# theartful/polychase

Measured on AMD Instinct MI355X. Metric: optical-flow frames/sec, higher is better.
Workload: dtype u8/int32 fixed-point + f32 2x2 solve; 1 GPU; C2 1920x1080 300-frame synthetic clip, 3-level pyramidal LK (max_level=3); width=1920, height=1080, max_level=3, window=10, pairs_per_frame=8, frames_per_gpu=1877, arith=opencv_x86, parallelism=single GPU

## Files before the change

### include/polychase_hip.h

```cpp
#ifndef POLYCHASE_HIP_H_
#define POLYCHASE_HIP_H_

#include <stddef.h>
#include <stdint.h>

#ifdef __cplusplus
extern "C" {
#endif

#define PC_OK 0
#define PC_E_INVALID (-1)
#define PC_E_NO_DEVICE (-2)
#define PC_E_HIP (-3)
#define PC_E_CAPACITY (-4)
#define PC_E_STATE (-5)

#define PC_MAX_TARGETS 8
#define PC_MAX_LEVELS 16
#define PC_MAX_WINDOW 31

typedef struct pc_context pc_context;
typedef struct pc_frame pc_frame;

typedef struct pc_gftt_options {
// ... 118 lines not shown
#define PC_ANALYZER_SPARE_SLOTS 3
#define PC_ANALYZER_LOOKAHEAD 1
int pc_analyzer_create(pc_context* ctx, int width, int height, const pc_gftt_options* gftt,
                       const pc_flow_options* flow, int ring_frames, int max_jobs, pc_analyzer** out);
void pc_analyzer_destroy(pc_analyzer* a);
int pc_analyzer_reset(pc_analyzer* a);
int pc_analyzer_put_frame(pc_analyzer* a, int32_t frame_id, const uint8_t* rgb, size_t row_pitch,
                          int on_device, int will_detect);
int pc_analyzer_put_frame_f32(pc_analyzer* a, int32_t frame_id, const float* rgb, size_t row_pitch, int channels,
                              int on_device, int will_detect);
int pc_analyzer_has_frame(const pc_analyzer* a, int32_t frame_id);
int pc_analyzer_frame_ingested(const pc_analyzer* a, int32_t frame_id);
int pc_analyzer_set_keypoints(pc_analyzer* a, int32_t frame_id, const float* xy, int n);
int pc_analyzer_submit(pc_analyzer* a, int32_t frame1, const int32_t* targets, int n_targets);
int pc_analyzer_pending(const pc_analyzer* a);
#define PC_LOG_MAGIC 0x50434c4f47303031ll
int pc_analyzer_set_device_log(pc_analyzer* a, void* d_log, size_t capacity_bytes);
int pc_analyzer_device_log_used(const pc_analyzer* a, size_t* bytes);
int pc_analyzer_redirect_device_log(pc_analyzer* a, void* d_log, size_t capacity_bytes);
int pc_analyzer_set_host_records(pc_analyzer* a, int enabled);
int pc_analyzer_set_fb_threshold(pc_analyzer* a, double fb_threshold);
int pc_analyzer_set_mask(pc_analyzer* a, const uint8_t* mask, size_t row_pitch, int on_device);
int pc_analyzer_set_mask_polygons(pc_analyzer* a, const float* xy, const int32_t* counts, int n_polygons, int invert);
int pc_analyzer_collect(pc_analyzer* a, pc_frame_result* out);

typedef struct pc_mesh pc_mesh;
typedef struct pc_pnp_problem pc_pnp_problem;

int pc_mesh_create(pc_context* ctx, const float* vertices, int n_vertices, const uint32_t* triangles,
                   int n_triangles, pc_mesh** out);
// ... 175 lines not shown
```

### polychase_amd/csrc/hip/api_analyzer.hip

```cpp
#include "api_internal.hpp"

using namespace pc_api;


namespace {

constexpr int kSpareSlots = PC_ANALYZER_SPARE_SLOTS;

enum DetState { DET_NONE = 0, DET_ENQUEUED = 2, DET_DONE = 3 };

struct Slot {
    pc_frame* frame = nullptr;
    int32_t frame_id = 0;
    bool valid = false;
    DetState det = DET_NONE;
    bool supplied = false;
    DetectScratch scratch;
    hipEvent_t last_read[2] = {nullptr, nullptr};
    hipEvent_t img_ready = nullptr;
    hipEvent_t kps_ready = nullptr;
};

struct Job {
    int32_t frame1 = 0;
    int n_kps = 0;
    bool detected = false;
    int n_targets = 0;
    int32_t targets[PC_MAX_TARGETS];
    PinBuf<uint8_t> h_pack;
    size_t o_kps = 0, o_idx = 0, o_xy = 0, o_err = 0, pack_bytes = 0;
    bool host_records = true;
    hipEvent_t done = nullptr;
};

struct HelperPriorityControl {
    static constexpr int kCalm = 48;
    static constexpr int kLagsToRaise = 3;
    int mode = -1;
    int hi = 0;
    int calm = 0;
    uint32_t window = 0;
    uint64_t lag_seen = 0, switched_on = 0;
    void init() {
        const char* v = getenv("POLYCHASE_HELPER_PRIO");
        mode = (v && (v[0] == '0' || v[0] == '1') && v[1] == 0) ? v[0] - '0' : -1;
        hi = mode == 1 ? 1 : 0;
    }
    void observe(bool lagging) {
        if (mode >= 0) return;
        window = ((window << 1) | (lagging ? 1u : 0u)) & 0xffffu;
        if (lagging) {
            lag_seen++;
            calm = 0;
            if (!hi && __builtin_popcount(window) >= kLagsToRaise) {
                hi = 1;
                switched_on++;
            }
        } else if (hi && ++calm >= kCalm) {
            hi = 0;
            calm = 0;
            window = 0;
        }
    }
};
struct HelperPriorityScope {
    explicit HelperPriorityScope(int hi) { pc::set_helper_prio(hi); }
    ~HelperPriorityScope() { pc::set_helper_prio(0); }
};

}

struct pc_analyzer {
    pc_context* ctx = nullptr;
    int w = 0, h = 0;
    pc_gftt_options gopt;
    pc_flow_options fopt;
    pc::GfttGrid grid;
    std::vector<Slot> slots;
    std::vector<Job> jobs;
    size_t job_head = 0, job_count = 0;
    uint64_t submitted = 0;
    bool one_lane = false;
    static constexpr int kLaneEvents = 16;
    hipEvent_t lk_done[2][kLaneEvents] = {};
    bool gate_armed = false;
    HelperPriorityControl prio;
    int32_t put_newest = 0, put_previous = 0;
    int puts = 0;
    bool host_records = true;
    double fb_threshold = 0.0;
    static constexpr int kMaskGens = 4;
    int mask_kind = 0;
    int mask_gen = 0;
    PinBuf<uint8_t> mask_host[kMaskGens];
    hipEvent_t mask_copied[kMaskGens] = {};
    const uint8_t* mask_dev = nullptr;
    size_t mask_dev_pitch = 0;
    int poly_gen = 0, poly_vertices = 0, poly_polygons = 0, poly_invert = 0;
    PinBuf<int32_t> poly_host[kMaskGens];
    DevBuf<int32_t> poly_dev[kMaskGens];
    hipEvent_t poly_read[kMaskGens] = {};
    uint8_t* d_log = nullptr;
    size_t log_cap = 0, log_used = 0;
// ... 8 lines not shown
    return (s.valid && s.frame_id == frame_id) ? &s : nullptr;
}

int detect_dense(pc_analyzer* a, Slot& s) {
    hipStream_t const ds = a->ctx->detect_stream_for(s.frame_id);
    PrepScope prep(a->ctx, ds);
    if (ds != a->ctx->prep_stream) PC_HIP(hipStreamWaitEvent(ds, s.img_ready, 0));
    int rc = detect_enqueue(a->ctx, s.frame, a->grid, a->gopt, s.scratch, s.scratch.bin_hist);
    if (rc != PC_OK) return rc;
    PC_HIP(hipEventRecord(s.kps_ready, ds));
    s.det = DET_ENQUEUED;
    s.supplied = false;
    return PC_OK;
}

int detect_finish_slot(pc_analyzer* a, Slot& s) {
    int rc;
    if (s.det == DET_NONE && (rc = detect_dense(a, s)) != PC_OK) return rc;
    {
        hipStream_t const ds = a->ctx->detect_stream_for(s.frame_id);
        PrepScope prep(a->ctx, ds);
        bool redone = false;
        if ((rc = detect_finish(a->ctx, s.frame, a->grid, a->gopt, s.scratch, s.scratch.bin_hist, &redone)) != PC_OK) return rc;
        if (redone) PC_HIP(hipEventRecord(s.kps_ready, ds));
    }
    s.det = DET_DONE;
    return PC_OK;
}

}

extern "C" {
// ... 7 lines not shown
    pc::GfttGrid grid0;
    {
        int vrc = validate_gftt(gftt, width, height, &grid0);
        if (vrc != PC_OK) return vrc;
    }
    PC_HIP(hipSetDevice(ctx->device));
    pc_analyzer* a = new (std::nothrow) pc_analyzer();
    if (!a) return fail(PC_E_INVALID, "out of host memory");
    a->ctx = ctx;
    a->one_lane = getenv("POLYCHASE_LK_LANES") && atoi(getenv("POLYCHASE_LK_LANES")) == 1;
    a->w = width;
    a->h = height;
    a->gopt = *gftt;
    a->fopt = *flow;
    a->grid = grid0;
    a->prio.init();
    a->slots.resize((size_t)ring_frames + kSpareSlots);
    a->jobs.resize((size_t)max_jobs);
    int rc = PC_OK;
    for (auto& s : a->slots) {
        rc = pc_frame_create(ctx, width, height, flow->window_size, flow->max_level, &s.frame);
        if (rc != PC_OK) break;
        const int kp0 = std::max(16384, (width * height) / 16);
        if ((rc = ensure_kp_capacity(s.frame, kp0)) != PC_OK) break;
        if (hipMalloc(reinterpret_cast<void**>(&s.frame->d_perm), (size_t)kp0 * 2 * sizeof(uint32_t)) != hipSuccess) {
            rc = fail(PC_E_HIP, "hipMalloc failed");
            break;
        }
        s.frame->perm_cap = kp0;
        if ((rc = detect_reserve(ctx, width, height, s.scratch, &a->gopt)) != PC_OK) break;
        if (s.scratch.bin_hist.ensure((size_t)pc::bin_num_tiles(width, height) + 1) != hipSuccess) {
// ... 81 lines not shown
    for (auto& s : a->slots) {
        s.valid = false;
        s.det = DET_NONE;
        s.supplied = false;
        s.frame_id = 0;
        s.last_read[0] = s.last_read[1] = nullptr;
        s.scratch.cleared = false;
        if (s.frame) s.frame->mask_on = false;
    }
    a->mask_kind = 0;
    a->mask_dev = nullptr;
    a->job_head = 0;
    a->d_log = nullptr;
    a->log_cap = a->log_used = 0;
    a->host_records = true;
    a->put_newest = a->put_previous = 0;
    a->puts = 0;
    a->prio = HelperPriorityControl();
    a->prio.init();
    return PC_OK;
}

static int analyzer_put(pc_analyzer* a, int32_t frame_id, const uint8_t* rgb, size_t row_pitch, int on_device,
                        int will_detect, int channels, int elem_size) {
    if (!a || !rgb) return fail(PC_E_INVALID, "null argument");
    const int n = (int)a->slots.size();
    Slot& s = a->slots[(size_t)(((frame_id % n) + n) % n)];
    PC_HIP(hipSetDevice(a->ctx->device));
    PrepScope prep(a->ctx);
    HelperPriorityScope prio_scope(a->prio.hi);
    a->put_previous = a->put_newest;
    a->put_newest = frame_id;
    a->puts++;
    for (hipEvent_t& e : s.last_read) {
        if (e) PC_HIP(hipStreamWaitEvent(a->ctx->prep_stream, e, 0));
        e = nullptr;
    }
    if (s.valid && s.det == DET_ENQUEUED && a->ctx->n_detect > 0) PC_HIP(hipStreamWaitEvent(a->ctx->prep_stream, s.kps_ready, 0));
    const bool clear_here = will_detect && a->ctx->n_detect == 0;
    int rc = set_image(a->ctx, s.frame, rgb, row_pitch, on_device, channels, elem_size, clear_here ? s.scratch.counters.p : nullptr,
                       detect_counter_words(s.scratch));
    s.scratch.cleared = rc == PC_OK && clear_here;
    if (rc != PC_OK) {
        s.valid = false;
        return rc;
    }
    s.frame->mask_on = false;
    if (will_detect && a->mask_kind == 1) {
// ... 1 lines not shown
        if ((rc = upload_mask(s.frame, a->mask_host[g].p, (size_t)a->w, PC_FRAME_PINNED_HOST, a->ctx->prep_stream)) != PC_OK) return rc;
        PC_HIP(hipEventRecord(a->mask_copied[g], a->ctx->prep_stream));
    } else if (will_detect && a->mask_kind == 2) {
        if ((rc = upload_mask(s.frame, a->mask_dev, a->mask_dev_pitch, 1, a->ctx->prep_stream)) != PC_OK) return rc;
    } else if (will_detect && a->mask_kind == 3) {
        const int g = a->poly_gen;
        if ((rc = fill_mask_polygons(s.frame, a->poly_dev[g].p, a->poly_vertices, a->poly_polygons, a->poly_invert, a->ctx->prep_stream)) != PC_OK)
            return rc;
        PC_HIP(hipEventRecord(a->poly_read[g], a->ctx->prep_stream));
    }
    PC_HIP(hipEventRecord(s.img_ready, a->ctx->prep_stream));
    s.frame_id = frame_id;
    s.valid = true;
    s.det = DET_NONE;
    s.supplied = false;
    if (will_detect) return detect_dense(a, s);
    return PC_OK;
}

int pc_analyzer_put_frame(pc_analyzer* a, int32_t frame_id, const uint8_t* rgb, size_t row_pitch, int on_device,
                          int will_detect) {
    return analyzer_put(a, frame_id, rgb, row_pitch, on_device, will_detect, 3, 1);
}

int pc_analyzer_put_frame_f32(pc_analyzer* a, int32_t frame_id, const float* rgb, size_t row_pitch, int channels,
                              int on_device, int will_detect) {
    return analyzer_put(a, frame_id, reinterpret_cast<const uint8_t*>(rgb), row_pitch, on_device, will_detect, channels, 4);
}

int pc_analyzer_has_frame(const pc_analyzer* a, int32_t frame_id) {
    if (!a) return 0;
    return find_slot(const_cast<pc_analyzer*>(a), frame_id) != nullptr;
}

int pc_analyzer_frame_ingested(const pc_analyzer* a, int32_t frame_id) {
    if (!a) return 1;
    Slot* s = find_slot(const_cast<pc_analyzer*>(a), frame_id);
    if (!s || !s->img_ready) return 1;
    return hipEventQuery(s->img_ready) == hipSuccess ? 1 : 0;
}

int pc_analyzer_set_keypoints(pc_analyzer* a, int32_t frame_id, const float* xy, int n) {
    if (!a || n < 0 || (!xy && n > 0)) return fail(PC_E_INVALID, "bad argument");
    Slot* s = find_slot(a, frame_id);
    if (!s) return fail(PC_E_STATE, "frame %d is not resident", frame_id);
    HelperPriorityScope prio_scope(a->prio.hi);
    int rc = ensure_kp_capacity(s->frame, n);
    if (rc != PC_OK) return rc;
    if (n > 0) {
        hipStream_t const ds = a->ctx->detect_stream_for(frame_id);
        PC_HIP(hipStreamSynchronize(ds));
        PC_HIP(hipMemcpyAsync(s->frame->d_kps, xy, (size_t)n * sizeof(float2), hipMemcpyHostToDevice, ds));
        PC_HIP(hipStreamSynchronize(ds));
    }
    s->frame->n_kps = n;
    {
        hipStream_t const ds = a->ctx->detect_stream_for(frame_id);
        PrepScope prep(a->ctx, ds);
        if ((rc = order_keypoints_spatially(a->ctx, s->frame, s->scratch.bin_hist)) != PC_OK) return rc;
        PC_HIP(hipEventRecord(s->kps_ready, ds));
    }
    s->det = DET_DONE;
    s->supplied = true;
    return PC_OK;
}


int pc_analyzer_submit(pc_analyzer* a, int32_t frame1, const int32_t* targets, int n_targets) {
    if (!a || (n_targets > 0 && !targets)) return fail(PC_E_INVALID, "null argument");
    if (n_targets < 0 || n_targets > PC_MAX_TARGETS) return fail(PC_E_INVALID, "n_targets must be in [0,%d]", PC_MAX_TARGETS);
    if (a->job_count == a->jobs.size()) return fail(PC_E_STATE, "%zu jobs already in flight: call pc_analyzer_collect", a->job_count);
    pc_context* ctx = a->ctx;
    PC_HIP(hipSetDevice(ctx->device));
    HelperPriorityScope prio_scope(a->prio.hi);
    Slot* s1 = find_slot(a, frame1);
    if (!s1) return fail(PC_E_STATE, "frame1 %d is not resident", frame1);
    const pc_frame* tg[PC_MAX_TARGETS];
    for (int t = 0; t < n_targets; t++) {
        Slot* st = find_slot(a, targets[t]);
        if (!st) return fail(PC_E_STATE, "target frame %d is not resident", targets[t]);
        tg[t] = st->frame;
    }
    int rc;
    bool detected = false;
    if (s1->det != DET_DONE) {
        SlowSection ss("submit/detect_finish");
        if ((rc = detect_finish_slot(a, *s1)) != PC_OK) return rc;
        detected = true;
    } else {
// ... 82 lines not shown
        hh[1] = frame1;
        hh[2] = n;
        hh[3] = n_targets;
        for (int t = 0; t < n_targets; t++) hh[4 + t] = targets[t];
        hh[12] = (long long)rows;
        PC_HIP(hipMemcpyAsync(a->d_log + o_hdr, hh, 128, hipMemcpyHostToDevice, ls));
        PC_HIP(hipMemcpyAsync(a->d_log + o_hdr + 128, pack, j.pack_bytes, hipMemcpyDeviceToDevice, ls));
        a->log_used = end;
    }
    a->submitted++;
    if (a->host_records) PC_HIP(hipMemcpyAsync(j.h_pack.p, pack, j.pack_bytes, hipMemcpyDeviceToHost, ls));
    else PC_HIP(hipMemcpyAsync(j.h_pack.p, pack, 128, hipMemcpyDeviceToHost, ls));
    j.host_records = a->host_records;
    PC_HIP(hipEventRecord(j.done, ls));
    a->job_count++;
    return PC_OK;
}

int pc_analyzer_pending(const pc_analyzer* a) { return a ? (int)a->job_count : 0; }

int pc_analyzer_set_device_log(pc_analyzer* a, void* d_log, size_t capacity_bytes) {
    if (!a) return fail(PC_E_INVALID, "null analyzer");
    if (d_log && (reinterpret_cast<uintptr_t>(d_log) & 15)) return fail(PC_E_INVALID, "device log must be 16-byte aligned");
    PC_HIP(a->ctx->sync_side_streams());
    PC_HIP(hipStreamSynchronize(a->ctx->stream));
    a->d_log = static_cast<uint8_t*>(d_log);
    a->log_cap = d_log ? capacity_bytes : 0;
    a->log_used = 0;
    return PC_OK;
}

int pc_analyzer_redirect_device_log(pc_analyzer* a, void* d_log, size_t capacity_bytes) {
    if (!a || !d_log) return fail(PC_E_INVALID, "null argument");
    if (reinterpret_cast<uintptr_t>(d_log) & 15) return fail(PC_E_INVALID, "device log must be 16-byte aligned");
// ... 72 lines not shown
    a->mask_dev = nullptr;
    return PC_OK;
}

int pc_analyzer_device_log_used(const pc_analyzer* a, size_t* bytes) {
    if (!a || !bytes) return fail(PC_E_INVALID, "null argument");
    *bytes = a->log_used;
    return PC_OK;
}

int pc_analyzer_collect(pc_analyzer* a, pc_frame_result* out) {
    if (!a || !out) return fail(PC_E_INVALID, "null argument");
    if (a->job_count == 0) return fail(PC_E_STATE, "no job in flight");
    Job& j = a->jobs[a->job_head];
    PC_HIP(hipEventSynchronize(j.done));
    if (a->puts >= 2) {
        Slot* const sp = find_slot(a, a->put_previous);
        bool lagging = sp && sp->img_ready && hipEventQuery(sp->img_ready) == hipErrorNotReady;
        if (a->ctx->n_detect > 0 && !lagging) {
            Slot* const sd = find_slot(a, j.frame1 + (int32_t)a->job_count + 1);
            lagging = sd && sd->det == DET_ENQUEUED && sd->kps_ready && hipEventQuery(sd->kps_ready) == hipErrorNotReady;
        }
        a->prio.observe(lagging);
    }
    (void)hipStreamQuery(a->ctx->stream);
    if (a->ctx->stream_b) (void)hipStreamQuery(a->ctx->stream_b);
    (void)hipStreamQuery(a->ctx->prep_stream);
    for (int k = 0; k < a->ctx->n_detect; k++) (void)hipStreamQuery(a->ctx->detect_stream[k]);
    out->frame1 = j.frame1;
    out->n_keypoints = j.n_kps;
    out->keypoints_detected = j.detected ? 1 : 0;
    out->keypoints_xy = j.host_records ? reinterpret_cast<const float*>(j.h_pack.p + j.o_kps) : nullptr;
    out->n_targets = j.n_targets;
    for (int t = 0; t < PC_MAX_TARGETS; t++) out->targets[t] = t < j.n_targets ? j.targets[t] : 0;
    const long long* h_ro = reinterpret_cast<const long long*>(j.h_pack.p);
    for (int t = 0; t <= PC_MAX_TARGETS; t++) out->row_offset[t] = (int64_t)h_ro[std::min(t, j.n_targets)];
    out->src_indices = j.host_records ? reinterpret_cast<const uint32_t*>(j.h_pack.p + j.o_idx) : nullptr;
    out->tgt_xy = j.host_records ? reinterpret_cast<const float*>(j.h_pack.p + j.o_xy) : nullptr;
// ... 8 lines not shown
```

### polychase_amd/csrc/hip/kernels.hpp

```cpp
#pragma once

#include "bvh.hpp"
#include "common.hpp"

namespace pc {

int helper_prio_arg();
void set_helper_prio(int hi);

void launch_rgb2gray(const uint8_t* rgb, size_t rgb_pitch, const Level& l0, hipStream_t s);
void launch_rgbf32_to_gray(const float* rgb, size_t rgb_pitch, int channels, const Level& l0, hipStream_t s);
void launch_copy_gray(const uint8_t* gray, size_t gray_pitch, const Level& l0, hipStream_t s);
void launch_pyrdown(const Level& src, const Level& dst, hipStream_t s);
void launch_border(const Level& l, int win, hipStream_t s);
void launch_widen(const Level& l, int win, hipStream_t s);
void launch_scharr(const Level& l, hipStream_t s);

enum LevelSourceKind { SRC_PYR = 0, SRC_RGB8 = 1, SRC_GRAY8 = 2, SRC_RGBF32 = 3 };
struct LevelSource {
    int kind;
    const uint8_t* src;
    size_t src_pitch;
    int channels;
    int aligned;
// ... 229 lines not shown
```

### polychase_amd/csrc/hip/kernels_gftt.hip

```cpp
#include <algorithm>
#include <cstring>
#include <type_traits>
#include <rocprim/device/device_radix_sort.hpp>

#include <cmath>

#include "kernels.hpp"

namespace pc {

constexpr int TW = 64, TH = 16;
constexpr int GH = TH + 4, G_PITCH = 72;
constexpr int CW = TW + 2, CH = TH + 2;

template <bool ROW_FMA>
__device__ __forceinline__ float smooth_row(float a, float b, float c, float f1, float f0) {
    float t = f1 * a;
    if (ROW_FMA) {
        t = __fmaf_rn(f0, b, t);
        t = __fmaf_rn(f1, c, t);
    } else {
        t += f0 * b;
        t += f1 * c;
    }
// ... 317 lines not shown

static int min_eig_variant() {
    static const int v = [] {
        const char* e = getenv("POLYCHASE_MINEIG_VARIANT");
        return e ? atoi(e) : 0;
    }();
    return v;
}

template <int SOBEL, bool MASKED>
static void launch_min_eig_masked(const Level& l0, float* eig, const GfttGrid& g, uint32_t* cell_max, float f1, float f0, hipStream_t s,
                                  const uint8_t* mask) {
    if (min_eig_variant() == 0) {
        dim3 grid2((l0.w + 2 * ME_TW - 1) / (2 * ME_TW), (l0.h + 2 * ME_TH - 1) / (2 * ME_TH));
        hipLaunchKernelGGL((min_eig_fused_kernel<SOBEL, MASKED>), grid2, dim3(256), 0, s, l0.img, l0.pitch, l0.w, l0.h, eig, g, cell_max, f1, f0,
                           helper_prio_arg(), mask);
        return;
    }
    dim3 grid((l0.w + TW - 1) / TW, (l0.h + TH - 1) / TH);
    hipLaunchKernelGGL((min_eig_kernel<SOBEL, MASKED>), grid, dim3(256), 0, s, l0.img, l0.pitch, l0.w, l0.h, eig, g, cell_max, f1, f0,
                       helper_prio_arg(), mask);
}
template <int SOBEL>
static void launch_min_eig_mode(const Level& l0, float* eig, const GfttGrid& g, uint32_t* cell_max, float f1, float f0, hipStream_t s,
                                const uint8_t* mask) {
    if (mask) launch_min_eig_masked<SOBEL, true>(l0, eig, g, cell_max, f1, f0, s, mask);
    else launch_min_eig_masked<SOBEL, false>(l0, eig, g, cell_max, f1, f0, s, nullptr);
}
void launch_min_eig(const Level& l0, float* eig, const GfttGrid& g, uint32_t* cell_max, int sobel_fma, hipStream_t s, const uint8_t* mask) {
    const double scale_d = 1.0 / (4.0 * 3.0 * 255.0);
    const float f1 = (float)(1.0 * scale_d), f0 = (float)(2.0 * scale_d);
    switch (sobel_fma & 3) {
        case 0: launch_min_eig_mode<0>(l0, eig, g, cell_max, f1, f0, s, mask); break;
        case 1: launch_min_eig_mode<1>(l0, eig, g, cell_max, f1, f0, s, mask); break;
        case 2: launch_min_eig_mode<2>(l0, eig, g, cell_max, f1, f0, s, mask); break;
        default: launch_min_eig_mode<3>(l0, eig, g, cell_max, f1, f0, s, mask); break;
// ... 149 lines not shown
#pragma unroll
        for (int d = 32; d >= 1; d >>= 1) key = max(key, (uint32_t)__shfl_xor((int)key, d));
        if ((threadIdx.x & 63) == (unsigned)(__ffsll((long long)__ballot(1)) - 1)) atomicMax(&cell_max[cell0], key);
    } else {
        atomicMax(&cell_max[cell], key);
    }
}

bool launch_corner_response(const Level& l0, float* eig, float* cov, double* box_rows, const GfttGrid& g, uint32_t* cell_max, int block_size, int gradient_size,
                            bool harris, double harris_k, int sobel_fma, hipStream_t s, const uint8_t* mask) {
    SobelTaps T;
    int taps = 0;
    if (!make_sobel_taps(gradient_size, block_size, &T, &taps)) return false;
    dim3 grid((l0.w + 63) / 64, (l0.h + 3) / 4);
    if (taps == 3)
        hipLaunchKernelGGL(cov_kernel<3>, grid, dim3(256), 0, s, l0.img, l0.pitch, l0.w, l0.h, cov, T, sobel_fma, helper_prio_arg());
    else if (taps == 5)
        hipLaunchKernelGGL(cov_kernel<5>, grid, dim3(256), 0, s, l0.img, l0.pitch, l0.w, l0.h, cov, T, sobel_fma, helper_prio_arg());
    else
        hipLaunchKernelGGL(cov_kernel<7>, grid, dim3(256), 0, s, l0.img, l0.pitch, l0.w, l0.h, cov, T, sobel_fma, helper_prio_arg());
    if (box_rows) hipLaunchKernelGGL(box_rows_kernel, grid, dim3(256), 0, s, cov, l0.w, l0.h, block_size, box_rows, helper_prio_arg());
    const int harris_mode = harris ? ((sobel_fma & 1) ? 2 : 1) : 0;
    if (mask)
        hipLaunchKernelGGL(box_response_kernel<true>, grid, dim3(256), 0, s, cov, (const double*)box_rows, l0.w, l0.h, block_size, harris_mode, harris_k, eig, g, cell_max,
                           helper_prio_arg(), mask);
    else
        hipLaunchKernelGGL(box_response_kernel<false>, grid, dim3(256), 0, s, cov, (const double*)box_rows, l0.w, l0.h, block_size, harris_mode, harris_k, eig, g, cell_max,
                           helper_prio_arg(), (const uint8_t*)nullptr);
    return true;
}

constexpr int NMS_SUB = 4;

struct SortRange {
    uint32_t hi, shift;
};
__host__ __device__ __forceinline__ SortRange make_sort_range(uint32_t lo, uint32_t hi) {
    SortRange r;
    r.hi = hi;
    r.shift = 0;
    const uint32_t span = hi > lo ? hi - lo : 0u;
    while ((span >> r.shift) >= (uint32_t)kSortBuckets) r.shift++;
    return r;
// ... 183 lines not shown
    if (ticket && last_workgroup(ticket, gridDim.x * gridDim.y)) {
        __shared__ uint32_t s_scan[256];
        const uint32_t total = scan_exclusive_256_fixed<kSortBuckets / 256>(hist, bucket_offsets, s_scan);
        if (tid == 0) bucket_offsets[kSortBuckets] = total;
    }
}

void launch_nms(const float* eig, int w, int h, const GfttGrid& g, const uint32_t* cell_max, double quality_level,
                unsigned long long* keys, uint32_t cap, uint32_t* counter, uint8_t* cstate, uint32_t* sort_params, uint32_t* hist,
                uint32_t* ticket, uint32_t* bucket_offsets, uint32_t* bin_hist, hipStream_t s,
                unsigned long long* slots, uint32_t* zero, int zero_words, const uint8_t* mask) {
    dim3 grid((w + TW - 1) / TW, (h + NMS_SUB * TH - 1) / (NMS_SUB * TH));
    if (mask)
        hipLaunchKernelGGL(nms_kernel<true>, grid, dim3(256), 0, s, eig, w, h, g, cell_max, quality_level, keys, cap, counter, cstate,
                           sort_params, hist, ticket, bucket_offsets, bin_hist, bin_hist ? bin_num_tiles(w, h) : 0, slots, zero,
                           zero ? zero_words : 0, helper_prio_arg(), mask);
    else
        hipLaunchKernelGGL(nms_kernel<false>, grid, dim3(256), 0, s, eig, w, h, g, cell_max, quality_level, keys, cap, counter, cstate,
                           sort_params, hist, ticket, bucket_offsets, bin_hist, bin_hist ? bin_num_tiles(w, h) : 0, slots, zero,
                           zero ? zero_words : 0, helper_prio_arg(), (const uint8_t*)nullptr);
}

constexpr int kBucketLds = 512;

__global__ __launch_bounds__(256) void bucket_scatter_kernel(const unsigned long long* __restrict__ keys, uint32_t cap,
                                                             const uint32_t* __restrict__ counter, const uint32_t* __restrict__ sort_params,
                                                             const uint32_t* __restrict__ offsets, uint32_t* __restrict__ cursor,
                                                             unsigned long long* __restrict__ out, int hi_prio) {
    helper_priority(hi_prio);
    const uint32_t n = min(*counter, cap);
    SortRange range;
    range.hi = sort_params[0];
    range.shift = sort_params[1];
    for (uint32_t i = blockIdx.x * blockDim.x + threadIdx.x; i < n; i += gridDim.x * blockDim.x) {
        const unsigned long long key = keys[i];
// ... 495 lines not shown
```

### polychase_amd/csrc/hip/kernels_pyramid.hip

```cpp
#include "kernels.hpp"

namespace pc {

static thread_local int tl_helper_prio = 0;
int helper_prio_arg() { return tl_helper_prio; }
void set_helper_prio(int hi) { tl_helper_prio = hi ? 1 : 0; }

namespace {

constexpr int TW = 64, TH = 16;
constexpr int CW = TW + 2, CH = TH + 2;
constexpr int C_X0 = 3;
constexpr int C_PITCH = 72;
constexpr int P_H = 2 * TH + 7;
constexpr int P_PITCH = 144;
constexpr int H_Q = (CW + 3) / 4;
constexpr int H_PITCH = 4 * H_Q;

__device__ __forceinline__ uint32_t gray_of(uint32_t r, uint32_t g, uint32_t b) {
    return (r * 9798u + g * 19235u + b * 3735u + (1u << 14)) >> 15;
}
__device__ __forceinline__ uint32_t float_channel_to_u8(float v) {
    const float s = v * 255.0f;
    const int i = (s >= -2147483648.0f && s < 2147483648.0f) ? (int)s : (int)0x80000000;
// ... 186 lines not shown
#pragma unroll
                for (int b = 0; b < 3; b++) {
                    if ((a | b) == 0 || my[a] == kNone || mx[b] == kNone) continue;
                    const ptrdiff_t o = (ptrdiff_t)my[a] * out.pitch + mx[b];
                    out.img[o] = (uint8_t)v;
                    out.img16[o] = (uint16_t)(v << 7);
                }
        }
    }
}

void launch_level(const LevelSource& in, const Level& out, int win, hipStream_t s) {
    dim3 grid((out.w + TW - 1) / TW, (out.h + TH - 1) / TH);
    switch (in.kind) {
        case SRC_PYR: hipLaunchKernelGGL(level_kernel<SRC_PYR>, grid, dim3(256), 0, s, in, out, win, helper_prio_arg()); break;
        case SRC_RGB8: hipLaunchKernelGGL(level_kernel<SRC_RGB8>, grid, dim3(256), 0, s, in, out, win, helper_prio_arg()); break;
        case SRC_GRAY8: hipLaunchKernelGGL(level_kernel<SRC_GRAY8>, grid, dim3(256), 0, s, in, out, win, helper_prio_arg()); break;
        default: hipLaunchKernelGGL(level_kernel<SRC_RGBF32>, grid, dim3(256), 0, s, in, out, win, helper_prio_arg()); break;
    }
}

}
```

### polychase_amd/hip.py

```python
from __future__ import annotations

import ctypes as C
import os

import numpy as np

from . import build as _build

PC_MAX_TARGETS = 8
KERNEL_CLASSES = ["gray", "pyramid", "min_eig", "nms", "sort", "suppress", "lk", "compact", "lk_fb"]

SYMBOLS = [
    "pc_gftt_default_options", "pc_flow_default_options", "pc_last_error", "pc_version",
    "pc_context_create", "pc_context_destroy", "pc_context_synchronize", "pc_context_stream",
    "pc_runtime_init", "pc_context_set_arithmetic", "pc_context_get_arithmetic", "pc_context_download",
    "pc_context_enable_timing", "pc_context_get_timing", "pc_context_get_busy_time", "pc_context_reset_timing",
    "pc_debug_lk_profile", "pc_debug_lk_x86_stats", "pc_debug_llt9",
    "pc_frame_create", "pc_frame_destroy", "pc_frame_set_rgb", "pc_frame_set_rgb_f32", "pc_frame_set_gray",
    "pc_host_buffer_alloc", "pc_host_buffer_free",
    "pc_frame_num_levels", "pc_frame_level_size", "pc_frame_download_gray", "pc_frame_download_level",
    "pc_frame_download_deriv", "pc_frame_detect", "pc_frame_download_min_eig", "pc_frame_num_candidates",
    "pc_frame_num_keypoints", "pc_frame_download_keypoints", "pc_frame_set_keypoints", "pc_frame_set_mask",
    "pc_frame_set_mask_polygons", "pc_frame_download_mask", "pc_analyzer_set_mask_polygons",
    "pc_lk_track", "pc_lk_track_filtered", "pc_lk_track_fb", "pc_lk_track_filtered_fb",
    "pc_analyzer_create", "pc_analyzer_destroy", "pc_analyzer_reset", "pc_analyzer_put_frame", "pc_analyzer_put_frame_f32",
    "pc_analyzer_has_frame", "pc_analyzer_frame_ingested",
    "pc_analyzer_set_keypoints", "pc_analyzer_submit", "pc_analyzer_pending", "pc_analyzer_collect",
    "pc_analyzer_set_device_log", "pc_analyzer_device_log_used", "pc_analyzer_redirect_device_log",
    "pc_analyzer_set_host_records", "pc_analyzer_set_fb_threshold", "pc_analyzer_set_mask",
    "pc_peer_buffer_alloc", "pc_peer_buffer_free", "pc_peer_buffer_export", "pc_peer_buffer_open", "pc_peer_buffer_close",
    "pc_peer_copy_async", "pc_peer_buffer_download",
    "pc_comm_unique_id", "pc_comm_create", "pc_comm_destroy", "pc_comm_world_size", "pc_comm_rank", "pc_comm_all_gather_log",
    "pc_comm_send", "pc_comm_recv",
    "pc_mesh_create", "pc_mesh_set_mask", "pc_mesh_destroy", "pc_raycast_pixels", "pc_raycast_pixels_sweep",
    "pc_corr_set_create", "pc_corr_set_destroy", "pc_corr_set_clear", "pc_corr_set_recycle", "pc_corr_set_append", "pc_corr_set_size",
    "pc_corr_set_download", "pc_pnp_problem_from_set",
    "pc_pnp_problem_create", "pc_pnp_problem_destroy", "pc_pnp_normal_equations", "pc_pnp_normal_equations_cost",
    "pc_pnp_solve", "pc_pnp_total_cost", "pc_track_solve_frame", "pc_track_frame_upload", "pc_track_frame_launch", "pc_track_frame_launch_chained", "pc_corr_set_reserve", "pc_context_pci_bus_id", "pc_track_frame_finish",
    "pc_track_download_points",
    "pc_refine_problem_create", "pc_refine_problem_create_parts", "pc_refine_problem_destroy", "pc_refine_total_cost", "pc_refine_normal_equations", "pc_refine_problem_timing",
]


ARITH_CANONICAL, ARITH_LK_X86_ORDER, ARITH_SOBEL_FMA, ARITH_OPENCV_X86 = 0, 1, 2, 3
# ... 5 lines not shown
                ("gradient_size", C.c_int), ("max_corners", C.c_int), ("use_harris", C.c_int),
                ("harris_k", C.c_double), ("grid_rows", C.c_int), ("grid_cols", C.c_int)]


class FlowOptions(C.Structure):
    _fields_ = [("window_size", C.c_int), ("max_level", C.c_int), ("term_max_iters", C.c_int),
                ("term_epsilon", C.c_double), ("min_eigen_threshold", C.c_double)]


class FrameResult(C.Structure):
    _fields_ = [("frame1", C.c_int32), ("n_keypoints", C.c_int32), ("keypoints_detected", C.c_int32),
                ("keypoints_xy", C.POINTER(C.c_float)), ("n_targets", C.c_int32),
                ("targets", C.c_int32 * 8), ("row_offset", C.c_int64 * 9),
                ("src_indices", C.POINTER(C.c_uint32)), ("tgt_xy", C.POINTER(C.c_float)),
                ("flow_err", C.POINTER(C.c_float))]


class PolychaseHipError(RuntimeError):
    pass


_lib = None


def load():
    global _lib
    if _lib is not None:
        return _lib
    path = _build.hip_library_path()
    if not os.path.exists(path):
# ... 58 lines not shown
    L.pc_analyzer_destroy.restype = None
    L.pc_analyzer_put_frame.argtypes = [vp, C.c_int32, vp, C.c_size_t, C.c_int, C.c_int]
    L.pc_analyzer_put_frame_f32.argtypes = [vp, C.c_int32, vp, C.c_size_t, C.c_int, C.c_int, C.c_int]
    L.pc_analyzer_has_frame.argtypes = [vp, C.c_int32]
    L.pc_analyzer_frame_ingested.argtypes = [vp, C.c_int32]
    L.pc_analyzer_set_keypoints.argtypes = [vp, C.c_int32, vp, C.c_int]
    L.pc_analyzer_submit.argtypes = [vp, C.c_int32, C.POINTER(C.c_int32), C.c_int]
    L.pc_analyzer_pending.argtypes = [vp]
    L.pc_analyzer_collect.argtypes = [vp, C.POINTER(FrameResult)]
    L.pc_analyzer_set_device_log.argtypes = [vp, vp, C.c_size_t]
    L.pc_analyzer_device_log_used.argtypes = [vp, C.POINTER(C.c_size_t)]
    L.pc_analyzer_reset.argtypes = [vp]
    L.pc_analyzer_redirect_device_log.argtypes = [vp, vp, C.c_size_t]
    L.pc_analyzer_set_host_records.argtypes = [vp, C.c_int]
    L.pc_analyzer_set_fb_threshold.argtypes = [vp, C.c_double]
    L.pc_analyzer_set_mask.argtypes = [vp, vp, C.c_size_t, C.c_int]
    L.pc_analyzer_set_mask_polygons.argtypes = [vp, vp, vp, C.c_int, C.c_int]
    L.pc_peer_buffer_alloc.argtypes = [C.c_int, C.c_size_t, C.POINTER(vp)]
    L.pc_peer_buffer_free.argtypes = [C.c_int, vp]
    L.pc_peer_buffer_export.argtypes = [C.c_int, vp, C.c_char_p]
    L.pc_peer_buffer_open.argtypes = [C.c_int, C.c_char_p, C.POINTER(vp)]
    L.pc_peer_buffer_close.argtypes = [C.c_int, vp]
    L.pc_peer_copy_async.argtypes = [C.c_int, vp, vp, C.c_size_t, vp]
    L.pc_peer_buffer_download.argtypes = [C.c_int, vp, vp, C.c_size_t]
    L.pc_comm_unique_id.argtypes = [vp]
    L.pc_comm_create.argtypes = [vp, vp, C.c_int, C.c_int, C.POINTER(vp)]
    L.pc_comm_destroy.argtypes = [vp]
    L.pc_comm_destroy.restype = None
    L.pc_comm_world_size.argtypes = [vp]
    L.pc_comm_rank.argtypes = [vp]
# ... 405 lines not shown
        keep, p, dev, pitch = _mask_ptr(mask, self.w, self.h)
        _check(load().pc_analyzer_set_mask(self._h, p, pitch, dev))
        self._keep_mask = keep if dev else None

    def set_mask_polygons(self, polys, invert: bool = False):
        xy, counts = _polygon_arrays(polys)
        _check(load().pc_analyzer_set_mask_polygons(self._h, xy.ctypes.data, counts.ctypes.data, len(counts), int(bool(invert))))
        self._keep_mask = None

    @property
    def device_log_used(self) -> int:
        n = C.c_size_t()
        _check(load().pc_analyzer_device_log_used(self._h, C.byref(n)))
        return n.value

    def collect_raw(self) -> FrameResult:
        r = FrameResult()
        _check(load().pc_analyzer_collect(self._h, C.byref(r)))
        return r

    def collect(self, copy: bool = True):
        r = self.collect_raw()
        n = r.n_keypoints
        if n and not r.keypoints_xy:
            return r.frame1, None, bool(r.keypoints_detected), {int(r.targets[t]): None for t in range(r.n_targets)}
        kps = np.ctypeslib.as_array(r.keypoints_xy, shape=(n, 2)) if n else np.zeros((0, 2), np.float32)
        flows = {}
        for t in range(r.n_targets):
            a, b = int(r.row_offset[t]), int(r.row_offset[t + 1])
            if b > a:
# ... 8 lines not shown
```

Before: 3439 frames/s.

## Split helper priority into narrow/bulk tiers and defer detection enqueue

Replaces the binary helper-priority controller with a three-state controller. Lag first raises only the narrow helper kernels (pyramid from a pyramid source) and only later the bulk kernels (GFTT cov/min-eig/NMS, full-resolution level build). Dense detection is no longer enqueued inside put_frame; it is deferred until the next put or until after a submit, so LK work for the current job gets launched ahead of it. Lag detection now checks two upcoming keypoint slots, and a stats query API is added. The deferred ordering may delay keypoint readiness, and the extra state adds control complexity.

```diff
diff --git a/include/polychase_hip.h b/include/polychase_hip.h
--- a/include/polychase_hip.h
+++ b/include/polychase_hip.h
@@ -156,6 +156,16 @@
 int pc_analyzer_set_keypoints(pc_analyzer* a, int32_t frame_id, const float* xy, int n);
 int pc_analyzer_submit(pc_analyzer* a, int32_t frame1, const int32_t* targets, int n_targets);
 int pc_analyzer_pending(const pc_analyzer* a);
+typedef struct {
+    int32_t mode;
+    int32_t state;
+    uint64_t collects;
+    uint64_t lag_pyramid;
+    uint64_t lag_keypoints;
+    uint64_t raises, lowers;
+    uint64_t collects_in_state[3];
+} pc_helper_priority_stats;
+int pc_analyzer_helper_priority_stats(const pc_analyzer* a, pc_helper_priority_stats* out);
 #define PC_LOG_MAGIC 0x50434c4f47303031ll
 int pc_analyzer_set_device_log(pc_analyzer* a, void* d_log, size_t capacity_bytes);
 int pc_analyzer_device_log_used(const pc_analyzer* a, size_t* bytes);
diff --git a/polychase_amd/csrc/hip/api_analyzer.hip b/polychase_amd/csrc/hip/api_analyzer.hip
--- a/polychase_amd/csrc/hip/api_analyzer.hip
+++ b/polychase_amd/csrc/hip/api_analyzer.hip
@@ -1,4 +1,5 @@
 #include "api_internal.hpp"
+#include "helper_priority_control.hpp"
 
 using namespace pc_api;
 
@@ -33,39 +34,10 @@
     hipEvent_t done = nullptr;
 };
 
-struct HelperPriorityControl {
-    static constexpr int kCalm = 48;
-    static constexpr int kLagsToRaise = 3;
-    int mode = -1;
-    int hi = 0;
-    int calm = 0;
-    uint32_t window = 0;
-    uint64_t lag_seen = 0, switched_on = 0;
-    void init() {
-        const char* v = getenv("POLYCHASE_HELPER_PRIO");
-        mode = (v && (v[0] == '0' || v[0] == '1') && v[1] == 0) ? v[0] - '0' : -1;
-        hi = mode == 1 ? 1 : 0;
-    }
-    void observe(bool lagging) {
-        if (mode >= 0) return;
-        window = ((window << 1) | (lagging ? 1u : 0u)) & 0xffffu;
-        if (lagging) {
-            lag_seen++;
-            calm = 0;
-            if (!hi && __builtin_popcount(window) >= kLagsToRaise) {
-                hi = 1;
-                switched_on++;
-            }
-        } else if (hi && ++calm >= kCalm) {
-            hi = 0;
-            calm = 0;
-            window = 0;
-        }
-    }
-};
+using pc::HelperPriorityControl;
 struct HelperPriorityScope {
-    explicit HelperPriorityScope(int hi) { pc::set_helper_prio(hi); }
-    ~HelperPriorityScope() { pc::set_helper_prio(0); }
+    explicit HelperPriorityScope(const HelperPriorityControl& c) { pc::set_helper_prio(c.priority(pc::kHelperNarrow), c.priority(pc::kHelperBulk)); }
+    ~HelperPriorityScope() { pc::set_helper_prio(0, 0); }
 };
 
 }
@@ -87,6 +59,8 @@
     HelperPriorityControl prio;
     int32_t put_newest = 0, put_previous = 0;
     int puts = 0;
+    int pending_det = -1;
+    bool put_since_submit = false;
     bool host_records = true;
     double fb_threshold = 0.0;
     static constexpr int kMaskGens = 4;
@@ -125,8 +99,20 @@
     return PC_OK;
 }
 
+int flush_pending_detection(pc_analyzer* a) {
+    if (a->pending_det < 0) return PC_OK;
+    Slot& s = a->slots[(size_t)a->pending_det];
+    a->pending_det = -1;
+    if (!s.valid || s.det != DET_NONE) return PC_OK;
+    return detect_dense(a, s);
+}
+void drop_pending_detection(pc_analyzer* a, const Slot& s) {
+    if (a->pending_det >= 0 && &a->slots[(size_t)a->pending_det] == &s) a->pending_det = -1;
+}
+
 int detect_finish_slot(pc_analyzer* a, Slot& s) {
     int rc;
+    drop_pending_detection(a, s);
     if (s.det == DET_NONE && (rc = detect_dense(a, s)) != PC_OK) return rc;
     {
         hipStream_t const ds = a->ctx->detect_stream_for(s.frame_id);
@@ -164,7 +150,7 @@
     a->gopt = *gftt;
     a->fopt = *flow;
     a->grid = grid0;
-    a->prio.init();
+    a->prio.init(getenv("POLYCHASE_HELPER_PRIO"));
     a->slots.resize((size_t)ring_frames + kSpareSlots);
     a->jobs.resize((size_t)max_jobs);
     int rc = PC_OK;
@@ -276,10 +262,11 @@
     a->d_log = nullptr;
     a->log_cap = a->log_used = 0;
     a->host_records = true;
+    a->pending_det = -1;
+    a->put_since_submit = false;
     a->put_newest = a->put_previous = 0;
     a->puts = 0;
-    a->prio = HelperPriorityControl();
-    a->prio.init();
+    a->prio.reset();
     return PC_OK;
 }
 
@@ -290,10 +277,12 @@
     Slot& s = a->slots[(size_t)(((frame_id % n) + n) % n)];
     PC_HIP(hipSetDevice(a->ctx->device));
     PrepScope prep(a->ctx);
-    HelperPriorityScope prio_scope(a->prio.hi);
+    HelperPriorityScope prio_scope(a->prio);
+    a->put_since_submit = true;
     a->put_previous = a->put_newest;
     a->put_newest = frame_id;
     a->puts++;
+    drop_pending_detection(a, s);
     for (hipEvent_t& e : s.last_read) {
         if (e) PC_HIP(hipStreamWaitEvent(a->ctx->prep_stream, e, 0));
         e = nullptr;
@@ -325,7 +314,8 @@
     s.valid = true;
     s.det = DET_NONE;
     s.supplied = false;
-    if (will_detect) return detect_dense(a, s);
+    if ((rc = flush_pending_detection(a)) != PC_OK) return rc;
+    if (will_detect) a->pending_det = (int)(&s - a->slots.data());
     return PC_OK;
 }
 
@@ -355,7 +345,8 @@
     if (!a || n < 0 || (!xy && n > 0)) return fail(PC_E_INVALID, "bad argument");
     Slot* s = find_slot(a, frame_id);
     if (!s) return fail(PC_E_STATE, "frame %d is not resident", frame_id);
-    HelperPriorityScope prio_scope(a->prio.hi);
+    HelperPriorityScope prio_scope(a->prio);
+    drop_pending_detection(a, *s);
     int rc = ensure_kp_capacity(s->frame, n);
     if (rc != PC_OK) return rc;
     if (n > 0) {
@@ -383,7 +374,7 @@
     if (a->job_count == a->jobs.size()) return fail(PC_E_STATE, "%zu jobs already in flight: call pc_analyzer_collect", a->job_count);
     pc_context* ctx = a->ctx;
     PC_HIP(hipSetDevice(ctx->device));
-    HelperPriorityScope prio_scope(a->prio.hi);
+    HelperPriorityScope prio_scope(a->prio);
     Slot* s1 = find_slot(a, frame1);
     if (!s1) return fail(PC_E_STATE, "frame1 %d is not resident", frame1);
     const pc_frame* tg[PC_MAX_TARGETS];
@@ -496,10 +487,26 @@
     j.host_records = a->host_records;
     PC_HIP(hipEventRecord(j.done, ls));
     a->job_count++;
+    if (!a->put_since_submit && (rc = flush_pending_detection(a)) != PC_OK) return rc;
+    a->put_since_submit = false;
     return PC_OK;
 }
 
 int pc_analyzer_pending(const pc_analyzer* a) { return a ? (int)a->job_count : 0; }
+
+int pc_analyzer_helper_priority_stats(const pc_analyzer* a, pc_helper_priority_stats* out) {
+    if (!a || !out) return fail(PC_E_INVALID, "null argument");
+    const HelperPriorityControl& c = a->prio;
+    out->mode = c.mode;
+    out->state = c.state;
+    out->collects = c.collects;
+    out->lag_pyramid = c.lag_pyramid;
+    out->lag_keypoints = c.lag_keypoints;
+    out->raises = c.raises;
+    out->lowers = c.lowers;
+    for (int k = 0; k < 3; k++) out->collects_in_state[k] = c.in_state[k];
+    return PC_OK;
+}
 
 int pc_analyzer_set_device_log(pc_analyzer* a, void* d_log, size_t capacity_bytes) {
     if (!a) return fail(PC_E_INVALID, "null analyzer");
@@ -602,14 +609,16 @@
     if (a->job_count == 0) return fail(PC_E_STATE, "no job in flight");
     Job& j = a->jobs[a->job_head];
     PC_HIP(hipEventSynchronize(j.done));
-    if (a->puts >= 2) {
-        Slot* const sp = find_slot(a, a->put_previous);
-        bool lagging = sp && sp->img_ready && hipEventQuery(sp->img_ready) == hipErrorNotReady;
-        if (a->ctx->n_detect > 0 && !lagging) {
-            Slot* const sd = find_slot(a, j.frame1 + (int32_t)a->job_count + 1);
-            lagging = sd && sd->det == DET_ENQUEUED && sd->kps_ready && hipEventQuery(sd->kps_ready) == hipErrorNotReady;
+    {
+        auto not_ready = [](hipEvent_t e) { return e && hipEventQuery(e) == hipErrorNotReady; };
+        Slot* const sp = a->puts >= 2 ? find_slot(a, a->put_previous) : nullptr;
+        const bool pyramid_late = sp && not_ready(sp->img_ready);
+        bool keypoints_late = false;
+        for (int k = 0; k < 2; k++) {
+            Slot* const sd = find_slot(a, j.frame1 + (int32_t)a->job_count + k);
+            keypoints_late = keypoints_late || (sd && sd->det == DET_ENQUEUED && not_ready(sd->kps_ready));
         }
-        a->prio.observe(lagging);
+        a->prio.observe(pyramid_late, keypoints_late);
     }
     (void)hipStreamQuery(a->ctx->stream);
     if (a->ctx->stream_b) (void)hipStreamQuery(a->ctx->stream_b);
diff --git a/polychase_amd/csrc/hip/helper_priority_control.hpp b/polychase_amd/csrc/hip/helper_priority_control.hpp
--- /dev/null
+++ b/polychase_amd/csrc/hip/helper_priority_control.hpp
@@ -0,0 +1,60 @@
+#pragma once
+
+#include <stdint.h>
+#include <string.h>
+
+namespace pc {
+
+enum HelperClass { kHelperNarrow = 0, kHelperBulk = 1 };
+
+struct HelperPriorityControl {
+    static constexpr int kCalm = 48;
+    static constexpr int kLagsToRaise = 3;
+    enum { kAllLow = 0, kNarrowHigh = 1, kAllHigh = 2 };
+    int mode = -1;
+    int state = kAllLow;
+    int calm = 0;
+    uint32_t window = 0;
+    uint64_t collects = 0, lag_pyramid = 0, lag_keypoints = 0, raises = 0, lowers = 0;
+    uint64_t in_state[3] = {0, 0, 0};
+
+    void init(const char* v) {
+        *this = HelperPriorityControl();
+        if (v && !strcmp(v, "0")) mode = kAllLow;
+        else if (v && !strcmp(v, "narrow")) mode = kNarrowHigh;
+        else if (v && !strcmp(v, "1")) mode = kAllHigh;
+        if (mode >= 0) state = mode;
+    }
+    void reset() {
+        const int m = mode;
+        *this = HelperPriorityControl();
+        mode = m;
+        if (mode >= 0) state = mode;
+    }
+    int priority(HelperClass c) const { return state >= (c == kHelperBulk ? kAllHigh : kNarrowHigh) ? 1 : 0; }
+
+    void observe(bool pyramid_late, bool keypoints_late) {
+        const bool lagging = pyramid_late || keypoints_late;
+        collects++;
+        in_state[state]++;
+        lag_pyramid += pyramid_late ? 1u : 0u;
+        lag_keypoints += keypoints_late ? 1u : 0u;
+        if (mode >= 0) return;
+        window = ((window << 1) | (lagging ? 1u : 0u)) & 0xffffu;
+        if (lagging) {
+            calm = 0;
+            if (state < kAllHigh && __builtin_popcount(window) >= kLagsToRaise) {
+                state++;
+                raises++;
+                window = 0;
+            }
+        } else if (state > kAllLow && ++calm >= kCalm) {
+            state--;
+            lowers++;
+            calm = 0;
+            window = 0;
+        }
+    }
+};
+
+}
diff --git a/polychase_amd/csrc/hip/kernels.hpp b/polychase_amd/csrc/hip/kernels.hpp
--- a/polychase_amd/csrc/hip/kernels.hpp
+++ b/polychase_amd/csrc/hip/kernels.hpp
@@ -6,7 +6,8 @@
 namespace pc {
 
 int helper_prio_arg();
-void set_helper_prio(int hi);
+int helper_prio_bulk_arg();
+void set_helper_prio(int narrow_hi, int bulk_hi);
 
 void launch_rgb2gray(const uint8_t* rgb, size_t rgb_pitch, const Level& l0, hipStream_t s);
 void launch_rgbf32_to_gray(const float* rgb, size_t rgb_pitch, int channels, const Level& l0, hipStream_t s);
diff --git a/polychase_amd/csrc/hip/kernels_gftt.hip b/polychase_amd/csrc/hip/kernels_gftt.hip
--- a/polychase_amd/csrc/hip/kernels_gftt.hip
+++ b/polychase_amd/csrc/hip/kernels_gftt.hip
@@ -355,12 +355,12 @@
     if (min_eig_variant() == 0) {
         dim3 grid2((l0.w + 2 * ME_TW - 1) / (2 * ME_TW), (l0.h + 2 * ME_TH - 1) / (2 * ME_TH));
         hipLaunchKernelGGL((min_eig_fused_kernel<SOBEL, MASKED>), grid2, dim3(256), 0, s, l0.img, l0.pitch, l0.w, l0.h, eig, g, cell_max, f1, f0,
-                           helper_prio_arg(), mask);
+                           helper_prio_bulk_arg(), mask);
         return;
     }
     dim3 grid((l0.w + TW - 1) / TW, (l0.h + TH - 1) / TH);
     hipLaunchKernelGGL((min_eig_kernel<SOBEL, MASKED>), grid, dim3(256), 0, s, l0.img, l0.pitch, l0.w, l0.h, eig, g, cell_max, f1, f0,
-                       helper_prio_arg(), mask);
+                       helper_prio_bulk_arg(), mask);
 }
 template <int SOBEL>
 static void launch_min_eig_mode(const Level& l0, float* eig, const GfttGrid& g, uint32_t* cell_max, float f1, float f0, hipStream_t s,
@@ -540,19 +540,19 @@
     if (!make_sobel_taps(gradient_size, block_size, &T, &taps)) return false;
     dim3 grid((l0.w + 63) / 64, (l0.h + 3) / 4);
     if (taps == 3)
-        hipLaunchKernelGGL(cov_kernel<3>, grid, dim3(256), 0, s, l0.img, l0.pitch, l0.w, l0.h, cov, T, sobel_fma, helper_prio_arg());
+        hipLaunchKernelGGL(cov_kernel<3>, grid, dim3(256), 0, s, l0.img, l0.pitch, l0.w, l0.h, cov, T, sobel_fma, helper_prio_bulk_arg());
     else if (taps == 5)
-        hipLaunchKernelGGL(cov_kernel<5>, grid, dim3(256), 0, s, l0.img, l0.pitch, l0.w, l0.h, cov, T, sobel_fma, helper_prio_arg());
+        hipLaunchKernelGGL(cov_kernel<5>, grid, dim3(256), 0, s, l0.img, l0.pitch, l0.w, l0.h, cov, T, sobel_fma, helper_prio_bulk_arg());
     else
-        hipLaunchKernelGGL(cov_kernel<7>, grid, dim3(256), 0, s, l0.img, l0.pitch, l0.w, l0.h, cov, T, sobel_fma, helper_prio_arg());
-    if (box_rows) hipLaunchKernelGGL(box_rows_kernel, grid, dim3(256), 0, s, cov, l0.w, l0.h, block_size, box_rows, helper_prio_arg());
+        hipLaunchKernelGGL(cov_kernel<7>, grid, dim3(256), 0, s, l0.img, l0.pitch, l0.w, l0.h, cov, T, sobel_fma, helper_prio_bulk_arg());
+    if (box_rows) hipLaunchKernelGGL(box_rows_kernel, grid, dim3(256), 0, s, cov, l0.w, l0.h, block_size, box_rows, helper_prio_bulk_arg());
     const int harris_mode = harris ? ((sobel_fma & 1) ? 2 : 1) : 0;
     if (mask)
         hipLaunchKernelGGL(box_response_kernel<true>, grid, dim3(256), 0, s, cov, (const double*)box_rows, l0.w, l0.h, block_size, harris_mode, harris_k, eig, g, cell_max,
-                           helper_prio_arg(), mask);
+                           helper_prio_bulk_arg(), mask);
     else
         hipLaunchKernelGGL(box_response_kernel<false>, grid, dim3(256), 0, s, cov, (const double*)box_rows, l0.w, l0.h, block_size, harris_mode, harris_k, eig, g, cell_max,
-                           helper_prio_arg(), (const uint8_t*)nullptr);
+                           helper_prio_bulk_arg(), (const uint8_t*)nullptr);
     return true;
 }
 
@@ -766,11 +766,11 @@
     if (mask)
         hipLaunchKernelGGL(nms_kernel<true>, grid, dim3(256), 0, s, eig, w, h, g, cell_max, quality_level, keys, cap, counter, cstate,
                            sort_params, hist, ticket, bucket_offsets, bin_hist, bin_hist ? bin_num_tiles(w, h) : 0, slots, zero,
-                           zero ? zero_words : 0, helper_prio_arg(), mask);
+                           zero ? zero_words : 0, helper_prio_bulk_arg(), mask);
     else
         hipLaunchKernelGGL(nms_kernel<false>, grid, dim3(256), 0, s, eig, w, h, g, cell_max, quality_level, keys, cap, counter, cstate,
                            sort_params, hist, ticket, bucket_offsets, bin_hist, bin_hist ? bin_num_tiles(w, h) : 0, slots, zero,
-                           zero ? zero_words : 0, helper_prio_arg(), (const uint8_t*)nullptr);
+                           zero ? zero_words : 0, helper_prio_bulk_arg(), (const uint8_t*)nullptr);
 }
 
 constexpr int kBucketLds = 512;
diff --git a/polychase_amd/csrc/hip/kernels_pyramid.hip b/polychase_amd/csrc/hip/kernels_pyramid.hip
--- a/polychase_amd/csrc/hip/kernels_pyramid.hip
+++ b/polychase_amd/csrc/hip/kernels_pyramid.hip
@@ -2,9 +2,13 @@
 
 namespace pc {
 
-static thread_local int tl_helper_prio = 0;
+static thread_local int tl_helper_prio = 0, tl_helper_prio_bulk = 0;
 int helper_prio_arg() { return tl_helper_prio; }
-void set_helper_prio(int hi) { tl_helper_prio = hi ? 1 : 0; }
+int helper_prio_bulk_arg() { return tl_helper_prio_bulk; }
+void set_helper_prio(int narrow_hi, int bulk_hi) {
+    tl_helper_prio = narrow_hi ? 1 : 0;
+    tl_helper_prio_bulk = bulk_hi ? 1 : 0;
+}
 
 namespace {
 
@@ -224,10 +228,10 @@
     dim3 grid((out.w + TW - 1) / TW, (out.h + TH - 1) / TH);
     switch (in.kind) {
         case SRC_PYR: hipLaunchKernelGGL(level_kernel<SRC_PYR>, grid, dim3(256), 0, s, in, out, win, helper_prio_arg()); break;
-        case SRC_RGB8: hipLaunchKernelGGL(level_kernel<SRC_RGB8>, grid, dim3(256), 0, s, in, out, win, helper_prio_arg()); break;
-        case SRC_GRAY8: hipLaunchKernelGGL(level_kernel<SRC_GRAY8>, grid, dim3(256), 0, s, in, out, win, helper_prio_arg()); break;
-        default: hipLaunchKernelGGL(level_kernel<SRC_RGBF32>, grid, dim3(256), 0, s, in, out, win, helper_prio_arg()); break;
-    }
-}
-
-}
+        case SRC_RGB8: hipLaunchKernelGGL(level_kernel<SRC_RGB8>, grid, dim3(256), 0, s, in, out, win, helper_prio_bulk_arg()); break;
+        case SRC_GRAY8: hipLaunchKernelGGL(level_kernel<SRC_GRAY8>, grid, dim3(256), 0, s, in, out, win, helper_prio_bulk_arg()); break;
+        default: hipLaunchKernelGGL(level_kernel<SRC_RGBF32>, grid, dim3(256), 0, s, in, out, win, helper_prio_bulk_arg()); break;
+    }
+}
+
+}
diff --git a/polychase_amd/hip.py b/polychase_amd/hip.py
--- a/polychase_amd/hip.py
+++ b/polychase_amd/hip.py
@@ -27,7 +27,7 @@
     "pc_analyzer_has_frame", "pc_analyzer_frame_ingested",
     "pc_analyzer_set_keypoints", "pc_analyzer_submit", "pc_analyzer_pending", "pc_analyzer_collect",
     "pc_analyzer_set_device_log", "pc_analyzer_device_log_used", "pc_analyzer_redirect_device_log",
-    "pc_analyzer_set_host_records", "pc_analyzer_set_fb_threshold", "pc_analyzer_set_mask",
+    "pc_analyzer_set_host_records", "pc_analyzer_set_fb_threshold", "pc_analyzer_set_mask", "pc_analyzer_helper_priority_stats",
     "pc_peer_buffer_alloc", "pc_peer_buffer_free", "pc_peer_buffer_export", "pc_peer_buffer_open", "pc_peer_buffer_close",
     "pc_peer_copy_async", "pc_peer_buffer_download",
     "pc_comm_unique_id", "pc_comm_create", "pc_comm_destroy", "pc_comm_world_size", "pc_comm_rank", "pc_comm_all_gather_log",
@@ -63,6 +63,12 @@
                 ("targets", C.c_int32 * 8), ("row_offset", C.c_int64 * 9),
                 ("src_indices", C.POINTER(C.c_uint32)), ("tgt_xy", C.POINTER(C.c_float)),
                 ("flow_err", C.POINTER(C.c_float))]
+
+
+class HelperPriorityStats(C.Structure):
+    _fields_ = [("mode", C.c_int32), ("state", C.c_int32), ("collects", C.c_uint64), ("lag_pyramid", C.c_uint64),
+                ("lag_keypoints", C.c_uint64), ("raises", C.c_uint64), ("lowers", C.c_uint64),
+                ("collects_in_state", C.c_uint64 * 3)]
 
 
 class PolychaseHipError(RuntimeError):
@@ -151,6 +157,7 @@
     L.pc_analyzer_redirect_device_log.argtypes = [vp, vp, C.c_size_t]
     L.pc_analyzer_set_host_records.argtypes = [vp, C.c_int]
     L.pc_analyzer_set_fb_threshold.argtypes = [vp, C.c_double]
+    L.pc_analyzer_helper_priority_stats.argtypes = [vp, C.POINTER(HelperPriorityStats)]
     L.pc_analyzer_set_mask.argtypes = [vp, vp, C.c_size_t, C.c_int]
     L.pc_analyzer_set_mask_polygons.argtypes = [vp, vp, vp, C.c_int, C.c_int]
     L.pc_peer_buffer_alloc.argtypes = [C.c_int, C.c_size_t, C.POINTER(vp)]
@@ -586,6 +593,13 @@
         _check(load().pc_analyzer_device_log_used(self._h, C.byref(n)))
         return n.value
 
+    def helper_priority_stats(self) -> dict:
+        st = HelperPriorityStats()
+        _check(load().pc_analyzer_helper_priority_stats(self._h, C.byref(st)))
+        return {"mode": "auto" if st.mode < 0 else int(st.mode), "state": int(st.state), "collects": int(st.collects),
+                "lag_pyramid": int(st.lag_pyramid), "lag_keypoints": int(st.lag_keypoints), "raises": int(st.raises),
+                "lowers": int(st.lowers), "collects_in_state": [int(x) for x in st.collects_in_state]}
+
     def collect_raw(self) -> FrameResult:
         r = FrameResult()
         _check(load().pc_analyzer_collect(self._h, C.byref(r)))
```

New measurement: 3467 frames/s, median of 6. No clear change (+0.8%).
